# NicoNeureiter/sBayes

Hardware: AMD Instinct MI355X
Metric: log-likelihood evals/sec at 1000 sites x 200 feats x 10 states; 1/2/4/8-GPU chains (higher is better)
Workload: dtype f64; 1 GPU; headline synthetic 1000x200x10, K=5, C=2 (BASELINE.json configs[2]); chains_per_gpu=4096, kernel=packed, log_mode=product, parallelism=1 independent engine(s), one per GPU, no collectives

## Files before the change

sbayes_amd/csrc/sbe_mixture_mfma.hip:

```cpp
#include <algorithm>
#include <cmath>
#include <cstdio>
#include <cstdlib>
#include <type_traits>
#include "sbe_mixture_mfma.hip.h"

#if defined(__HIP_DEVICE_COMPILE__) && !defined(__gfx950__) && !defined(__gfx942__)
#error "sbe_mixture_mfma.hip: the in-kernel final reduction orders relaxed agent-scope atomics by s_waitcnt (gfx942 / gfx950 cache behaviour); not valid for this target"
#endif

namespace sbe {

constexpr int kMfmaRN = kTupleMfmaColsPerPass;

__global__ void k_xt_frags(const uint8_t* __restrict__ state , uint8_t* __restrict__ xt,
                           int N, int F, int S, int Fp, int NT, int KBp) {
    const int64_t u = (int64_t)blockIdx.x * blockDim.x + threadIdx.x;
    if (u >= (int64_t)NT * KBp * 64) return;
    const int l = (int)(u & 63), kb = (int)((u >> 6) % KBp), nt = (int)((u >> 6) / KBp);
    const int col = nt * 32 + (l & 31), f = col / S, s = col - f * S;
    uint32_t w[4] = {0u, 0u, 0u, 0u};
    if (col < F * S) {
        const int n0 = kb * 64 + 32 * (l >> 5);
#pragma unroll
        for (int j = 0; j < 32; ++j) {
            const int n = n0 + 8 * (j >> 3) + (j & 7);
            const int b = j & 3, hi = (j >> 2) & 1;
            if (n < N && state[(int64_t)n * Fp + f] == (uint8_t)s) w[j >> 3] |= 0x2u << (8 * b + 4 * hi);
        }
    }
    reinterpret_cast<uint4*>(xt)[u] = make_uint4(w[0], w[1], w[2], w[3]);
}

__global__ void k_colcount(const uint8_t* __restrict__ state, int32_t* __restrict__ colcount, int32_t* __restrict__ colfeat,
                           int N, int F, int S, int Fp, int NT) {
    const int col = (int)(blockIdx.x * blockDim.x + threadIdx.x);
    if (col >= (NT + 1) * 32) return;
    int c = 0;
    const int f = min(col / S, F - 1);
    if (col < F * S) {
        const int s = col - f * S;
        for (int n = 0; n < N; ++n) c += state[(int64_t)n * Fp + f] == (uint8_t)s;
    }
    colcount[col] = c;
    colfeat[col] = f;
}

__global__ void k_tile_prefix(const int32_t* __restrict__ colcount, int32_t* __restrict__ tile_prefix, int NT) {
    if (threadIdx.x != 0 || blockIdx.x != 0) return;
    int acc = 0;
    for (int t = 0; t <= NT + 1; ++t) {
        tile_prefix[t] = acc;
        if (t <= NT) for (int i = 0; i < 32; ++i) acc += colcount[t * 32 + i];
    }
}

size_t column_tables_bytes(int NT) { return ((size_t)(NT + 1) * 64 + (size_t)NT + 2) * sizeof(int32_t); }
void launch_column_tables(const uint8_t* state, int32_t* out, int N, int F, int S, int Fp, int NT, hipStream_t st) {
    int32_t* colcount = out;
    int32_t* colfeat = out + (size_t)(NT + 1) * 32;
    int32_t* tile_prefix = out + (size_t)(NT + 1) * 64;
    k_colcount<<<(unsigned)(((NT + 1) * 32 + 255) / 256), 256, 0, st>>>(state, colcount, colfeat, N, F, S, Fp, NT);
    k_tile_prefix<<<1, 64, 0, st>>>(colcount, tile_prefix, NT);
}

void launch_xt_frags(const uint8_t* state, uint8_t* xt, int N, int F, int S, int Fp, int NT, int KBp, hipStream_t st) {
    const int64_t units = (int64_t)NT * KBp * 64;
    k_xt_frags<<<(unsigned)((units + 255) / 256), 256, 0, st>>>(state, xt, N, F, S, Fp, NT, KBp);
}

void fine_log_table(double* tab ) {
    for (int i = 0; i < kFineLogEntries; ++i) {
        const long double c = i == 0 ? 1.0L : i == kFineLogEntries - 1 ? 2.0L : 1.0L + (i + 0.5L) / kFineLogEntries;
        const double inv_c = (double)(1.0L / c);
        const long double lc = -logl((long double)inv_c) - (i >= kFineLogSplit ? logl(2.0L) : 0.0L);
        tab[2 * i] = 0.5 * inv_c;
        tab[2 * i + 1] = (i == 0 || i == kFineLogEntries - 1) ? 0.0 : (double)lc;
    }
}

template <int MT, int CT, int GT = 4, int SLB = 4, bool SHARE = false>
__global__ __launch_bounds__(kMfmaThreads, 1) void k_mixture_tuple_mfma(MfmaMixParams p) {
    typedef v16f_t acc_t;
    constexpr int SL = 1 << SLB, TPT = 32 / SL, TPB = MT * TPT;
    constexpr int NK = SL == 16 ? 8 : SL;
    extern __shared__ __align__(16) unsigned char lds_raw[];
    const int lane = threadIdx.x & (kWave - 1);
    const int w = __builtin_amdgcn_readfirstlane((int)(threadIdx.x >> 6));
    const int split = (int)blockIdx.x % p.n_split, sg = (int)blockIdx.x / p.n_split;
    const int KBp = p.KBp;
    constexpr uint32_t tab_off = 0u;
    constexpr uint32_t a_off = kFineLogEntries * 16u;
    const uint32_t a_bytes = (uint32_t)MT * (uint32_t)KBp * 1024u;
    const uint32_t meta_off = a_off + a_bytes;
    const uint32_t red_off = meta_off + (uint32_t)(SL * TPB * sizeof(TupleMeta<CT>));
    const uint32_t lds_base = (uint32_t)(uintptr_t)(__attribute__((address_space(3))) unsigned char*)lds_raw;
    typedef TupleMeta<CT> Meta;
    Meta* meta = reinterpret_cast<Meta*>(lds_raw + meta_off);
    double* red = reinterpret_cast<double*>(lds_raw + red_off);

    auto slot_of = [&](int sl) -> int {
        const int i = sg * SL + sl;
        if (i >= p.n_batch) return -1;
        return p.slot_list ? p.slot_list[i] : p.first_slot + i;
    };

    const int nt_lo = split * p.nt_per_split, nt_hi = min(p.NT, nt_lo + p.nt_per_split);
    constexpr int PF = 4;
    const __amdgpu_buffer_rsrc_t xt_rsrc = __builtin_amdgcn_make_buffer_rsrc(const_cast<uint8_t*>(p.xt), 0, (int)p.xt_bytes, 0x00020000);
    const int lane16 = lane * 16;
    auto tile_off = [&](int nt) -> int { return (nt < nt_hi ? nt : p.NT) * KBp * 1024; };
    auto load_b = [&](int toff, int kb) -> v4i_t {
        const u32x4_t d = __builtin_amdgcn_raw_buffer_load_b128(xt_rsrc, lane16, toff + kb * 1024, 0);
        v4i_t r; r.x = (int)d.x; r.y = (int)d.y; r.z = (int)d.z; r.w = (int)d.w;
        return r;
    };
    v4i_t bq[PF][kMfmaRN];
    {
        const int nt0 = nt_lo + w * kMfmaRN;
#pragma unroll
        for (int i = 0; i < PF; ++i)
#pragma unroll
            for (int r = 0; r < kMfmaRN; ++r) bq[i][r] = load_b(tile_off(nt0 + r), i);
    }

    if (lds_base != 0u) {
        if ((int)threadIdx.x < SL) {
            const int slot = slot_of((int)threadIdx.x);
            if (slot >= 0) {
                p.partials[(int64_t)slot * p.partials_stride + split] = __longlong_as_double(0x7FF8000000000000ll);
                if (p.results) p.results[slot] = __longlong_as_double(0x7FF8000000000000ll);
            }
        }
        return;
    }
    static_assert(!SHARE || (SL == 16 && CT == 2 && MT <= 3), "the shared-operand epilogue: 16 slots, C = 2, <= 6 tuples");
    const uint4* sdesc = reinterpret_cast<const uint4*>(lds_raw + meta_off);
    const uint4* tdesc = reinterpret_cast<const uint4*>(lds_raw + meta_off + SL * 16);
    const int slot_mine = slot_of((int)threadIdx.x & (SL - 1));
    SharedDescIn<SHARE ? TPB : 1> sd_in;
    if constexpr (SHARE) mfma_shared_desc_load<MT, SL>(p, slot_mine, sd_in);
    mfma_phase0<MT, CT, decltype(slot_of), SL, !SHARE>(lds_raw, p, slot_of, tab_off, a_off, meta, KBp, slot_mine);
    if constexpr (SHARE) mfma_shared_desc<MT, SL>(p, sd_in, const_cast<uint4*>(sdesc), const_cast<uint4*>(tdesc));
    __syncthreads();
    bool bad = false;
    if constexpr (SHARE) bad = __builtin_amdgcn_ballot_w64(sdesc[lane & (SL - 1)].w != 0u) != 0ull;

    const int h = lane >> 5, cl = lane & 31;
    double lsum[NK];
    int ksum[NK];
#pragma unroll
    for (int i = 0; i < NK; ++i) { lsum[i] = 0.0; ksum[i] = 0; }
    auto ent_slot = [&](int e) -> int { return ((e & 3) + 8 * (e >> 2) + 4 * h) & (SL - 1); };
    auto ent_tuple = [&](int m, int e) -> int { return m * TPT + (((e & 3) + 8 * (e >> 2) + 4 * h) >> SLB); };
    auto ent_k = [&](int e) -> int { return SL == 16 ? (e & 3) + 4 * ((e >> 2) & 1) : (e & (SL - 1)); };
    int csum = 0;
    uint32_t one_hi = 0x3FF00000u;
    asm volatile("" : "+v"(one_hi));
    const __amdgpu_buffer_rsrc_t pr_rsrc = __builtin_amdgcn_make_buffer_rsrc(const_cast<float*>(p.probs), 0, (int)p.probs_bytes, 0x00020000);
    const __amdgpu_buffer_rsrc_t w_rsrc = __builtin_amdgcn_make_buffer_rsrc(const_cast<float*>(p.wpat), 0, (int)p.wpat_bytes, 0x00020000);
    const uint32_t a_lane = a_off + (uint32_t)lane * 16u;

    auto counts_pass = [&](acc_t (&acc)[MT][kMfmaRN], const int (&toff)[kMfmaRN]) __attribute__((always_inline)) {
        uint32_t a_at[MT];
        v4i_t a_cur[MT];
#pragma unroll
        for (int m = 0; m < MT; ++m) {
            a_at[m] = a_lane + ((uint32_t)m * (uint32_t)KBp) * 1024u;
            asm volatile("" : "+v"(a_at[m]));
            a_cur[m] = *(lds_cv4i_t*)(uintptr_t)a_at[m];
        }
        auto k_group = [&](int kb0, auto first_c) __attribute__((always_inline)) {
            constexpr bool first = decltype(first_c)::value;
#pragma unroll
            for (int i = 0; i < PF; ++i) {
                v4i_t a_nxt[MT];
#pragma unroll
                for (int m = 0; m < MT; ++m) a_nxt[m] = *(lds_cv4i_t*)(uintptr_t)(a_at[m] + (uint32_t)(i + 1) * 1024u);
                const bool refill = !(first && i == 0);
                if (refill) {
#pragma unroll
                    for (int r = 0; r < kMfmaRN; ++r) bq[(i + PF - 1) % PF][r] = load_b(toff[r], kb0 + i + PF - 1);
                }
#pragma unroll
                for (int m = 0; m < MT; ++m)
#pragma unroll
                    for (int r = 0; r < kMfmaRN; ++r) {
                        const v4i_t bx = bq[i][r];
                        const v8i_t a8 = {a_cur[m].x, a_cur[m].y, a_cur[m].z, a_cur[m].w, 0, 0, 0, 0};
                        const v8i_t b8 = {bx.x, bx.y, bx.z, bx.w, 0, 0, 0, 0};
                        const acc_t zero = {0, 0, 0, 0, 0, 0, 0, 0, 0, 0, 0, 0, 0, 0, 0, 0};
                        if (first && i == 0) acc[m][r] = __builtin_amdgcn_mfma_scale_f32_32x32x64_f8f6f4(a8, b8, zero, 4, 4, 0, 0, 0, 0);
                        else acc[m][r] = __builtin_amdgcn_mfma_scale_f32_32x32x64_f8f6f4(a8, b8, acc[m][r], 4, 4, 0, 0, 0, 0);
                    }
#pragma unroll
                for (int m = 0; m < MT; ++m) a_cur[m] = a_nxt[m];
                __builtin_amdgcn_sched_group_barrier(0x100, MT, 0);
                if (refill) __builtin_amdgcn_sched_group_barrier(0x020, kMfmaRN, 0);
                __builtin_amdgcn_sched_group_barrier(0x008, MT * kMfmaRN, 0);
            }
#pragma unroll
            for (int m = 0; m < MT; ++m) a_at[m] += (uint32_t)PF * 1024u;
        };
        k_group(0, std::true_type{});
        for (int kb0 = PF; kb0 < KBp; kb0 += PF) k_group(kb0, std::false_type{});
    };

    constexpr int G = GT;
    constexpr int HQ = 4 / G;
    constexpr int NST = MT * 4 * HQ * kMfmaRN;
    uint32_t col4[kMfmaRN], fw4[kMfmaRN];
    Meta mdq[G];
    float prq[2][G][CT], wrq[2][G][CT];
    auto st_cols = [&](int nt0) {
#pragma unroll
        for (int r = 0; r < kMfmaRN; ++r) {
            const uint32_t colc = (uint32_t)min((nt0 + r) * 32 + cl, p.FS - 1);
            const uint32_t f = colc / (uint32_t)p.S;
            col4[r] = colc * 4u; fw4[r] = f * (uint32_t)(CT * 4);
        }
    };
    auto st_meta = [&](int u) {
        const int mj = u / HQ, half = u % HQ, m = mj >> 2, j = mj & 3;
#pragma unroll
        for (int i = 0; i < G; ++i) {
            const int e = 4 * j + half * G + i;
            mdq[i] = meta[ent_slot(e) * TPB + ent_tuple(m, e)];
        }
    };
    auto st_load = [&](int q) {
        const int r = q % kMfmaRN;
#pragma unroll
        for (int i = 0; i < G; ++i) {
            const uint32_t wo = mdq[i].woff + fw4[r];
            if constexpr (CT == 2) {
                const u32x2_t v2 = __builtin_amdgcn_raw_buffer_load_b64(w_rsrc, (int)wo, 0, 0);
                const uint32_t e0 = v2.x, e1 = v2.y;
                wrq[q & 1][i][0] = __uint_as_float(e0); wrq[q & 1][i][1] = __uint_as_float(e1);
            } else if constexpr (CT == 4) {
                const u32x4_t v4 = __builtin_amdgcn_raw_buffer_load_b128(w_rsrc, (int)wo, 0, 0);
                const uint32_t e0 = v4.x, e1 = v4.y, e2 = v4.z, e3 = v4.w;
                wrq[q & 1][i][0] = __uint_as_float(e0); wrq[q & 1][i][1] = __uint_as_float(e1);
                wrq[q & 1][i][2] = __uint_as_float(e2); wrq[q & 1][i][3] = __uint_as_float(e3);
            } else {
#pragma unroll
                for (int c = 0; c < CT; ++c)
                    wrq[q & 1][i][c] = __builtin_bit_cast(float, __builtin_amdgcn_raw_buffer_load_b32(w_rsrc, (int)(wo + 4u * c), 0, 0));
            }
#pragma unroll
            for (int c = 0; c < CT; ++c)
                prq[q & 1][i][c] = __builtin_bit_cast(float, __builtin_amdgcn_raw_buffer_load_b32(pr_rsrc, (int)(mdq[i].goff[c] + col4[r]), 0, 0));
        }
    };
    auto st_comp = [&](int q, const acc_t (&acc)[MT][kMfmaRN]) __attribute__((always_inline)) {
        const int r = q % kMfmaRN, u = q / kMfmaRN, mj = u / HQ, half = u % HQ, m = mj >> 2, j = mj & 3;
        double vv[G], lg[G], cntd[G];
        int cnt[G];
        bool special = false;
#pragma unroll
        for (int i = 0; i < G; ++i) {
            const float c = acc[m][r][4 * j + half * G + i];
            cnt[i] = (int)c; cntd[i] = (double)c;
            double v = 0.0;
#pragma unroll
            for (int c = 0; c < CT; ++c) {
                const double wc = (double)wrq[q & 1][i][c], pc = (double)prq[q & 1][i][c];
                v = c == 0 ? wc * pc : fma(wc, pc, v);
            }
            vv[i] = v;
            special |= __builtin_amdgcn_class(v, 0x2FF);
        }
        int kx[G];
        tab_log4_n<G>(vv, lg, kx, tab_off, one_hi);
        if (__builtin_expect(__builtin_amdgcn_ballot_w64(special) != 0ull, 0)) {
#pragma unroll
            for (int i = 0; i < G; ++i)
                if (__builtin_amdgcn_class(vv[i], 0x2FF)) { lg[i] = cnt[i] != 0 ? lib_log(vv[i]) : 0.0; kx[i] = kFineLogBias; }
        }
#pragma unroll
        for (int i = 0; i < G; ++i) {
            const int k = ent_k(4 * j + half * G + i);
            lsum[k] = fma(cntd[i], lg[i], lsum[k]);
            ksum[k] = __mul24(cnt[i], kx[i]) + ksum[k];
            asm volatile("" : "+v"(ksum[k]));
            asm volatile("" : "+v"(lsum[k]));
        }
    };

    constexpr int NSS = 8 * MT;
    uint32_t sh_col4[kMfmaRN], sh_fw4[kMfmaRN], col4u = 0;
    uint4 sdq, tdq[2];
    float p0q[2][4], p1r[kMfmaRN];
    uint32_t wr[kMfmaRN][4];
    uint64_t selm[2][2];
    double w0a[kMfmaRN], ua[kMfmaRN], w0b[kMfmaRN], ub[kMfmaRN];
    auto k_slot = [&](int k) -> int { return (k & 3) + 8 * (k >> 2) + 4 * h; };
    auto sh_desc = [&](int k) { sdq = sdesc[k_slot(k)]; };
    auto sh_load = [&]() {
#pragma unroll
        for (int r = 0; r < kMfmaRN; ++r) {
            p1r[r] = __builtin_bit_cast(float, __builtin_amdgcn_raw_buffer_load_b32(pr_rsrc, (int)(sdq.x + sh_col4[r]), 0, 0));
            const u32x2_t va = __builtin_amdgcn_raw_buffer_load_b64(w_rsrc, (int)(sdq.y + sh_fw4[r]), 0, 0);
            const u32x2_t vb = __builtin_amdgcn_raw_buffer_load_b64(w_rsrc, (int)(sdq.z + sh_fw4[r]), 0, 0);
            const uint32_t a0 = va.x, a1 = va.y, b0 = vb.x, b1 = vb.y;
            wr[r][0] = a0; wr[r][1] = a1; wr[r][2] = b0; wr[r][3] = b1;
        }
    };
    auto sh_conv = [&]() {
#pragma unroll
        for (int r = 0; r < kMfmaRN; ++r) {
            const double p1 = (double)p1r[r];
            w0a[r] = (double)__uint_as_float(wr[r][0]); ua[r] = (double)__uint_as_float(wr[r][1]) * p1;
            w0b[r] = (double)__uint_as_float(wr[r][2]); ub[r] = (double)__uint_as_float(wr[r][3]) * p1;
        }
    };
    auto td_read = [&](int q) { tdq[q & 1] = tdesc[k_slot(q / MT) * MT + q % MT]; };
    auto p0_load = [&](int q) {
        const uint4 d = tdq[q & 1];
        const uint32_t o0 = d.x + col4u, o1 = d.y + col4u;
        p0q[q & 1][0] = __builtin_bit_cast(float, __builtin_amdgcn_raw_buffer_load_b32(pr_rsrc, (int)o0, 0, 0));
        p0q[q & 1][1] = __builtin_bit_cast(float, __builtin_amdgcn_raw_buffer_load_b32(pr_rsrc, (int)(o0 + 128u), 0, 0));
        p0q[q & 1][2] = __builtin_bit_cast(float, __builtin_amdgcn_raw_buffer_load_b32(pr_rsrc, (int)o1, 0, 0));
        p0q[q & 1][3] = __builtin_bit_cast(float, __builtin_amdgcn_raw_buffer_load_b32(pr_rsrc, (int)(o1 + 128u), 0, 0));
        selm[q & 1][0] = __builtin_amdgcn_ballot_w64(d.z != 0u);
        selm[q & 1][1] = __builtin_amdgcn_ballot_w64(d.w != 0u);
    };
    auto sh_comp = [&](int q, const acc_t (&acc)[MT][kMfmaRN]) __attribute__((always_inline)) {
        const int k = q / MT, m = q % MT;
        double vv[4], lg[4], cntd[4];
        int cnt[4];
        bool special = false;
#pragma unroll
        for (int i = 0; i < 4; ++i) {
            const int tt = i >> 1, r = i & 1;
            const float c = acc[m][r][4 * ((k >> 2) + 2 * tt) + (k & 3)];
            cnt[i] = (int)c; cntd[i] = (double)c;
            const double p0 = (double)p0q[q & 1][i];
            double v = fma(w0a[r], p0, ua[r]);
            uint64_t keep;
            asm("s_and_saveexec_b64 %1, %2\n\tv_fma_f64 %0, %3, %4, %5\n\ts_mov_b64 exec, %1"
                : "+v"(v), "=&s"(keep) : "s"(selm[q & 1][tt]), "v"(w0b[r]), "v"(p0), "v"(ub[r]) : "scc");
            vv[i] = v;
            special |= __builtin_amdgcn_class(v, 0x2FF);
        }
        int kx[4];
        tab_log4_n<4>(vv, lg, kx, tab_off, one_hi);
        if (__builtin_expect(__builtin_amdgcn_ballot_w64(special) != 0ull, 0)) {
#pragma unroll
            for (int i = 0; i < 4; ++i)
                if (__builtin_amdgcn_class(vv[i], 0x2FF)) { lg[i] = cnt[i] != 0 ? lib_log(vv[i]) : 0.0; kx[i] = kFineLogBias; }
        }
#pragma unroll
        for (int i = 0; i < 4; ++i) {
            lsum[k] = fma(cntd[i], lg[i], lsum[k]);
            ksum[k] = __mul24(cnt[i], kx[i]) + ksum[k];
            asm volatile("" : "+v"(ksum[k]));
            asm volatile("" : "+v"(lsum[k]));
        }
    };

    const __amdgpu_buffer_rsrc_t cc_rsrc = __builtin_amdgcn_make_buffer_rsrc(const_cast<int32_t*>(p.colcount), 0, (p.NT + 1) * 128, 0x00020000);
    auto load_cc = [&](int nt) -> int { return (int)__builtin_amdgcn_raw_buffer_load_b32(cc_rsrc, cl * 4, (nt < nt_hi ? nt : p.NT) * 128, 0); };
    int ccnt[kMfmaRN];
    for (int nt0 = nt_lo + w * kMfmaRN; nt0 < nt_hi; nt0 += kMfmaWaves * kMfmaRN) {
        int toff[kMfmaRN];
#pragma unroll
        for (int r = 0; r < kMfmaRN; ++r) toff[r] = tile_off(nt0 + r);
        const bool first_pass = nt0 == nt_lo + w * kMfmaRN;
        if (!first_pass) {
#pragma unroll
            for (int i = 0; i < PF; ++i)
#pragma unroll
                for (int r = 0; r < kMfmaRN; ++r) bq[i][r] = load_b(toff[r], i);
        }
        if (first_pass) {
#pragma unroll
            for (int r = 0; r < kMfmaRN; ++r) ccnt[r] = load_cc(nt0 + r);
        }
        acc_t acc[MT][kMfmaRN];
        counts_pass(acc, toff);
#pragma unroll
        for (int r = 0; r < kMfmaRN; ++r) {
            csum += ccnt[r];
            ccnt[r] = load_cc(nt0 + kMfmaWaves * kMfmaRN + r);
        }
        if constexpr (SHARE) {
#pragma unroll
            for (int r = 0; r < kMfmaRN; ++r) {
                const uint32_t colc = (uint32_t)min((nt0 + r) * 32 + cl, p.FS - 1);
                sh_col4[r] = colc * 4u; sh_fw4[r] = colc / (uint32_t)p.S * (uint32_t)(CT * 4);
            }
            col4u = (uint32_t)(nt0 * 32 + cl) * 4u;
            sh_desc(0); td_read(0); td_read(1);
            sh_load();
            p0_load(0);
#pragma unroll
            for (int q = 0; q < NSS; ++q) {
                const int k = q / MT, m = q % MT;
                if (m == 0) {
                    sh_conv();
                    if (k + 1 < 8) sh_desc(k + 1);
                }
                if (m == (MT > 1 ? 1 : 0) && k + 1 < 8) sh_load();
                if (q + 1 < NSS) {
                    p0_load(q + 1);
                    if (q + 2 < NSS) td_read(q + 2);
                }
                sh_comp(q, acc);
                __builtin_amdgcn_sched_barrier(0);
            }
        } else {
        st_cols(nt0);
        st_meta(0);
        st_load(0);
#pragma unroll
        for (int q = 0; q < NST; ++q) {
            if (q + 1 < NST) {
                st_load(q + 1);
                if ((q + 2) % kMfmaRN == 0 && q + 2 < NST) st_meta((q + 2) / kMfmaRN);
            }
            st_comp(q, acc);
            __builtin_amdgcn_sched_barrier(0);
        }
        }
    }

#pragma unroll
    for (int i = 0; i < NK; ++i) {
        double v;
        if constexpr (SL == 16) {
            v = fma((double)(ksum[i] - kFineLogBias * csum), 6.93147180559945286227e-01, lsum[i]);
        } else {
            const int ks = ksum[i] + __shfl_xor(ksum[i], 32, 64);
            v = h == 0 ? fma((double)(ks - kFineLogBias * csum), 6.93147180559945286227e-01, lsum[i]) : lsum[i];
        }
#pragma unroll
        for (int off = 16; off >= 1; off >>= 1) v += __shfl_xor(v, off, 64);
        lsum[i] = v;
    }
    if (cl == 0) {
#pragma unroll
        for (int i = 0; i < NK; ++i) {
            if constexpr (SL == 16) {
                const int sl = 8 * (i >> 2) + 4 * h + (i & 3);
                red[(w * 2 + h) * 16 + sl] = lsum[i];
                red[(w * 2 + h) * 16 + (sl ^ 4)] = 0.0;
            } else {
                red[(w * 2 + h) * 16 + i] = lsum[i];
            }
        }
    }
    __syncthreads();
    if (w != 0) return;
    const int my_slot = lane < SL ? slot_of(lane) : -1;
    double total = 0.0;
    if (my_slot >= 0) {
#pragma unroll
        for (int ww = 0; ww < kMfmaWaves; ++ww) { total += red[(ww * 2 + 0) * 16 + lane]; total += red[(ww * 2 + 1) * 16 + lane]; }
    }
    if (bad) total = __longlong_as_double(0x7FF8000000000000ll);
    double* const my_partials = p.partials + (int64_t)max(my_slot, 0) * p.partials_stride;
    if (!p.results) {
        if (my_slot >= 0) my_partials[split] = total;
        return;
    }
    if (p.n_split > 1) {
        if (my_slot >= 0) __hip_atomic_store(my_partials + split, total, __ATOMIC_RELAXED, __HIP_MEMORY_SCOPE_AGENT);
        asm volatile("s_waitcnt vmcnt(0)" ::: "memory");
        unsigned t = 0;
        if (lane == 0) {
            t = __hip_atomic_fetch_add(p.arrive + sg, 1u, __ATOMIC_RELAXED, __HIP_MEMORY_SCOPE_AGENT);
            if (t == (unsigned)p.n_split - 1u) __hip_atomic_store(p.arrive + sg, 0u, __ATOMIC_RELAXED, __HIP_MEMORY_SCOPE_AGENT);
        }
        t = (unsigned)__builtin_amdgcn_readfirstlane((int)t);
        if (t != (unsigned)p.n_split - 1u) return;
        asm volatile("" ::: "memory");
        if (my_slot >= 0) {
            total = 0.0;
            for (int k = 0; k < p.n_split; ++k) total += __hip_atomic_load(my_partials + k, __ATOMIC_RELAXED, __HIP_MEMORY_SCOPE_AGENT);
        }
    }
    if (my_slot >= 0) p.results[my_slot] = total;
    signal_done(p.done);
}

template <int MT, int CT> constexpr int mfma_gt() { return (MT >= 4 || (MT == 3 && CT >= 3)) ? 2 : 4; }

template <int MT, int SLB>
static void launch_mfma_mt(int C, const MfmaMixParams& p, dim3 grid, size_t lds, hipStream_t st) {
    switch (C) {
        case 1: k_mixture_tuple_mfma<MT, 1, mfma_gt<MT, 1>(), SLB><<<grid, kMfmaThreads, lds, st>>>(p); break;
        case 2:
            if constexpr (SLB == 4 && MT <= 3) {
                if (p.shared) { k_mixture_tuple_mfma<MT, 2, mfma_gt<MT, 2>(), SLB, true><<<grid, kMfmaThreads, lds, st>>>(p); break; }
            }
            k_mixture_tuple_mfma<MT, 2, mfma_gt<MT, 2>(), SLB><<<grid, kMfmaThreads, lds, st>>>(p);
            break;
        case 3: k_mixture_tuple_mfma<MT, 3, mfma_gt<MT, 3>(), SLB><<<grid, kMfmaThreads, lds, st>>>(p); break;
        default: k_mixture_tuple_mfma<MT, 4, mfma_gt<MT, 4>(), SLB><<<grid, kMfmaThreads, lds, st>>>(p); break;
    }
}

template <int MT, int CT, int SLB, bool SHARE = false>
static bool allow_lds() {
    const void* fn = reinterpret_cast<const void*>(&k_mixture_tuple_mfma<MT, CT, mfma_gt<MT, CT>(), SLB, SHARE>);
    (void)hipFuncSetAttribute(fn, hipFuncAttributeMaxDynamicSharedMemorySize, (int)kLdsBytes);
    hipFuncAttributes attr{};
    if (hipFuncGetAttributes(&attr, fn) != hipSuccess) { (void)hipGetLastError(); return true; }
    return attr.sharedSizeBytes == 0;
}

template <int SLB>
static bool allow_lds_all() {
    bool ok = true;
    ok &= allow_lds<1, 1, SLB>(); ok &= allow_lds<1, 2, SLB>(); ok &= allow_lds<1, 3, SLB>(); ok &= allow_lds<1, 4, SLB>();
    ok &= allow_lds<2, 1, SLB>(); ok &= allow_lds<2, 2, SLB>(); ok &= allow_lds<2, 3, SLB>(); ok &= allow_lds<2, 4, SLB>();
    ok &= allow_lds<3, 1, SLB>(); ok &= allow_lds<3, 2, SLB>(); ok &= allow_lds<3, 3, SLB>(); ok &= allow_lds<3, 4, SLB>();
    ok &= allow_lds<4, 1, SLB>(); ok &= allow_lds<4, 2, SLB>(); ok &= allow_lds<4, 3, SLB>(); ok &= allow_lds<4, 4, SLB>();
    if constexpr (SLB == 4) {
        ok &= allow_lds<1, 2, SLB, true>(); ok &= allow_lds<2, 2, SLB, true>(); ok &= allow_lds<3, 2, SLB, true>();
    }
    return ok;
}

bool tuple_mfma_shared() {
    static const bool on = [] { const char* v = getenv("SBE_MFMA_SHARED"); return !(v && atoi(v) == 0); }();
    return on;
}

template <int SLB>
static void launch_mfma_slb(int MT, int C, const MfmaMixParams& p, dim3 grid, size_t lds, hipStream_t st) {
    switch (MT) {
        case 1: launch_mfma_mt<1, SLB>(C, p, grid, lds, st); break;
        case 2: launch_mfma_mt<2, SLB>(C, p, grid, lds, st); break;
        case 3: launch_mfma_mt<3, SLB>(C, p, grid, lds, st); break;
        default: launch_mfma_mt<4, SLB>(C, p, grid, lds, st); break;
    }
}

bool launch_tuple_mfma(int C, const MfmaMixParams& p, dim3 grid, size_t lds, hipStream_t st) {
    static const bool no_static_lds = [] { bool ok = allow_lds_all<4>(); ok &= allow_lds_all<2>(); ok &= allow_lds_all<1>(); return ok; }();
    if (!no_static_lds) return false;
    const int SL = p.SL;
    const int MT = (p.KT + 32 / SL - 1) / (32 / SL);
    if (SL == 16) launch_mfma_slb<4>(MT, C, p, grid, lds, st);
    else if (SL == 4) launch_mfma_slb<2>(MT, C, p, grid, lds, st);
    else launch_mfma_slb<1>(MT, C, p, grid, lds, st);
    return true;
}

}
```

sbayes_amd/csrc/sbe_mixture_mfma.hip.h:

```cpp
#pragma once
#include "sbe_mixture.hip.h"

namespace sbe {

typedef int v4i_t __attribute__((ext_vector_type(4)));
typedef int v8i_t __attribute__((ext_vector_type(8)));
typedef float v16f_t __attribute__((ext_vector_type(16)));
typedef __attribute__((address_space(3))) const v4i_t lds_cv4i_t;

constexpr int kMfmaSlots = 16;
constexpr int kMfmaThreads = kMfmaWaves * kWave;

constexpr int kFineLogSplit = 424;
constexpr uint32_t kFineLogCarry = 0x00100000u - ((uint32_t)kFineLogSplit << 10);
constexpr int kFineLogBias = 1023;
template <int G>
__device__ __forceinline__ void tab_log4_n(const double (&v)[G], double (&out)[G], int (&kexp)[G], uint32_t tab, uint32_t one_hi ) {
    f64x2_t e[G];
    double m[G], r[G], q[G];
    uint32_t mant_mask = 0x000FFFFFu;
    asm volatile("" : "+s"(mant_mask));
#pragma unroll
    for (int g = 0; g < G; ++g) {
        const uint32_t hi = (uint32_t)__double2hiint(v[g]);
        e[g] = *(lds_cf64x2_t*)(uintptr_t)(tab + ((hi >> 6) & 0x3FF0u));
        uint32_t mh;
        asm("v_bfi_b32 %0, %1, %2, %3" : "=v"(mh) : "s"(mant_mask), "v"(hi), "v"(one_hi));
        m[g] = __hiloint2double((int)mh, __double2loint(v[g]));
        kexp[g] = (int)((hi + kFineLogCarry) >> 20);
    }
#pragma unroll
    for (int g = 0; g < G; ++g) r[g] = fma(m[g], e[g].x, -0.5);
#pragma unroll
    for (int g = 0; g < G; ++g) q[g] = fma(r[g], -4.0, 8.0 / 3.0);
#pragma unroll
    for (int g = 0; g < G; ++g) q[g] = fma(r[g], q[g], -2.0);
#pragma unroll
    for (int g = 0; g < G; ++g) q[g] = fma(r[g], q[g], 2.0);
#pragma unroll
    for (int g = 0; g < G; ++g) out[g] = fma(r[g], q[g], e[g].y);
}

template <int CT>
struct __attribute__((aligned(CT <= 1 ? 8 : (CT <= 3 ? 16 : 32)))) TupleMeta {
    uint32_t woff;
    uint32_t goff[CT];
};

template <int MT, int CT, typename SlotOf, int SL = kMfmaSlots, bool META = true>
__device__ __forceinline__ void mfma_phase0(unsigned char* lds_raw, const MfmaMixParams& p, const SlotOf& slot_of, uint32_t tab_off,
                                            uint32_t a_off, TupleMeta<CT>* meta, int KBp, int slot_mine) {
    typedef TupleMeta<CT> Meta;
    constexpr int TPT = 32 / SL, TPB = MT * TPT;
    static_assert(SL == 16 || SL == 4 || SL == 2, "slots per block");
    static_assert(kMfmaThreads % SL == 0, "a thread's id units all belong to one slot");
    auto meta_of = [&](int slot, int t, uint32_t pat, const uint32_t (&g)[CT]) -> Meta {
        Meta md;
        md.woff = p.wpat_ones_off;
#pragma unroll
        for (int c = 0; c < CT; ++c) md.goff[c] = p.probs_ones_off;
        if (slot >= 0 && t < p.KT && pat != 0xFFu) {
            md.woff = (uint32_t)(((int64_t)slot * p.wpat_stride + (int64_t)pat * p.F * CT) * 4);
#pragma unroll
            for (int c = 0; c < CT; ++c)
                if ((int)g[c] < p.Gtot) md.goff[c] = (uint32_t)(((int64_t)slot * p.probs_stride + (int64_t)g[c] * p.FS) * 4);
        }
        return md;
    };
    constexpr bool PERM = TPB <= 8;
    constexpr uint32_t kNoTuple = PERM ? 0x0C0C0C0Cu : 0xFFFFFFFFu;
    const int n_units = SL * KBp * 2;
    constexpr int UB = 2;
    uint32_t d[UB][8];
    auto load_ids = [&](int u0) {
#pragma unroll
        for (int k = 0; k < UB; ++k) {
            const int u = u0 + k * kMfmaThreads;
            const int n0 = (u / SL) * 32;
            const int slot = u < n_units ? slot_mine : -1;
#pragma unroll
            for (int i = 0; i < 8; ++i) {
                d[k][i] = kNoTuple;
                if (slot >= 0 && n0 + 4 * i + 4 <= p.Np)
                    d[k][i] = *reinterpret_cast<const uint32_t*>(p.tid + (int64_t)slot * p.tid_stride + n0 + 4 * i);
            }
        }
    };
    auto emit = [&](int u0) {
#pragma unroll
        for (int k = 0; k < UB; ++k) {
            const int u = u0 + k * kMfmaThreads;
            if (u >= n_units) break;
            const int sl = u % SL, hk = u / SL;
            const int kb = hk >> 1, h = hk & 1;
#pragma unroll 8
            for (int t = 0; t < TPB; ++t) {
                uint4 o;
                uint32_t* ov = reinterpret_cast<uint32_t*>(&o);
#pragma unroll
                for (int wv = 0; wv < 4; ++wv) {
                    if constexpr (PERM) {
                        const uint64_t lut = 0x02ull << (8 * (t & 7));
                        const uint32_t lo = __builtin_amdgcn_perm((uint32_t)(lut >> 32), (uint32_t)lut, d[k][2 * wv]);
                        const uint32_t hi = __builtin_amdgcn_perm((uint32_t)(lut >> 32), (uint32_t)lut, d[k][2 * wv + 1]);
                        ov[wv] = lo | (hi << 4);
                        continue;
                    }
                    uint32_t eq[2];
#pragma unroll
                    for (int q = 0; q < 2; ++q) {
                        const uint32_t x = d[k][2 * wv + q] ^ ((uint32_t)t * 0x01010101u);
                        const uint32_t nz = ((x & 0x7F7F7F7Fu) + 0x7F7F7F7Fu) | x;
                        eq[q] = (~nz >> 7) & 0x01010101u;
                    }
                    ov[wv] = (eq[0] << 1) | (eq[1] << 5);
                }
                const uint32_t fl = (uint32_t)(h * 32 + (t % TPT) * SL + sl);
                *reinterpret_cast<uint4*>(lds_raw + a_off + (((uint32_t)(t / TPT) * (uint32_t)KBp + (uint32_t)kb) * 64u + fl) * 16u) = o;
            }
        }
    };
    const int u_first = (int)threadIdx.x;
    load_ids(u_first);
    constexpr int LT = (2 * kFineLogEntries + kMfmaThreads - 1) / kMfmaThreads;
    double lt[LT];
#pragma unroll
    for (int k = 0; k < LT; ++k) {
        const int i = (int)threadIdx.x + k * kMfmaThreads;
        lt[k] = i < 2 * kFineLogEntries ? reinterpret_cast<const double*>(p.logtab)[i] : 0.0;
    }
    const bool has_meta = META && (int)threadIdx.x < SL * TPB;
    const int m_sl = (int)threadIdx.x / TPB, m_t = (int)threadIdx.x % TPB;
    const int m_slot = has_meta ? slot_of(m_sl) : -1;
    uint32_t m_pat = 0xFFu, m_g[CT];
#pragma unroll
    for (int c = 0; c < CT; ++c) m_g[c] = 0xFFFFFFFFu;
    if (m_slot >= 0) {
        m_pat = p.tuple_p[(int64_t)m_slot * p.tuple_p_stride + m_t];
#pragma unroll
        for (int c = 0; c < CT; ++c) m_g[c] = p.tuple_g[(int64_t)m_slot * p.tuple_g_stride + m_t * kMaxComponents + c];
    }
    if (has_meta) meta[m_sl * TPB + m_t] = meta_of(m_slot, m_t, m_pat, m_g);
    (void)meta;
#pragma unroll
    for (int k = 0; k < LT; ++k) {
        const int i = (int)threadIdx.x + k * kMfmaThreads;
        if (i < 2 * kFineLogEntries) reinterpret_cast<double*>(lds_raw + tab_off)[i] = lt[k];
    }
    for (int u0 = u_first; u0 < n_units; u0 += UB * kMfmaThreads) {
        if (u0 != u_first) load_ids(u0);
        emit(u0);
    }
}

template <int TPB>
struct SharedDescIn {
    int slot;
    uint32_t pat[TPB], g0[TPB], g1[TPB];
};

template <int MT, int SL>
__device__ __forceinline__ void mfma_shared_desc_load(const MfmaMixParams& p, int slot, SharedDescIn<MT * 32 / SL>& in) {
    constexpr int TPB = MT * 32 / SL;
    static_assert(SL == 16 && TPB <= kMaxTuples, "the shared-operand form has 16 slots of <= 8 tuples");
    if ((int)threadIdx.x >= SL) return;
    in.slot = slot;
    const uint8_t* const tp = p.tuple_p + (int64_t)max(slot, 0) * p.tuple_p_stride;
    const uint16_t* const tg = p.tuple_g + (int64_t)max(slot, 0) * p.tuple_g_stride;
#pragma unroll
    for (int t = 0; t < TPB; ++t) {
        in.pat[t] = tp[t];
        in.g0[t] = tg[t * kMaxComponents + 0];
        in.g1[t] = tg[t * kMaxComponents + 1];
    }
}

template <int MT, int SL>
__device__ __forceinline__ void mfma_shared_desc(const MfmaMixParams& p, const SharedDescIn<MT * 32 / SL>& in, uint4* sdesc, uint4* tdesc) {
    constexpr int TPB = MT * 32 / SL;
    if ((int)threadIdx.x >= SL) return;
    const int sl = (int)threadIdx.x, slot = in.slot;
    const uint32_t (&g0)[TPB] = in.g0, (&g1)[TPB] = in.g1;
    uint32_t pat[TPB];
#pragma unroll
    for (int t = 0; t < TPB; ++t) pat[t] = (slot >= 0 && t < p.KT) ? in.pat[t] : 0xFFu;
    auto goff = [&](uint32_t g) -> uint32_t {
        return (int)g < p.Gtot ? (uint32_t)(((int64_t)slot * p.probs_stride + (int64_t)g * p.FS) * 4) : p.probs_ones_off;
    };
    uint32_t goff1 = p.probs_ones_off, wa = p.wpat_ones_off, wb = p.wpat_ones_off, bad = 0u;
    uint32_t go0[TPB], sel[TPB];
    bool any = false;
#pragma unroll
    for (int t = 0; t < TPB; ++t) {
        go0[t] = p.probs_ones_off; sel[t] = 0u;
        if (pat[t] == 0xFFu) continue;
        go0[t] = goff(g0[t]);
        const uint32_t wo = (uint32_t)(((int64_t)slot * p.wpat_stride + (int64_t)pat[t] * p.F * 2) * 4), g1o = goff(g1[t]);
        if (!any) { any = true; goff1 = g1o; wa = wb = wo; }
        if (g1o != goff1) bad = 1u;
        if (wo != wa) {
            if (wb == wa) wb = wo;
            else if (wo != wb) bad = 1u;
            sel[t] = 1u;
        }
    }
    sdesc[sl] = make_uint4(goff1, wa, wb, bad);
#pragma unroll
    for (int m = 0; m < MT; ++m) tdesc[sl * MT + m] = make_uint4(go0[2 * m], go0[2 * m + 1], sel[2 * m], sel[2 * m + 1]);
}

}
```

Measured before the change: 76.79 million evals/s.

## Split epilogue log into LDS lookup and series stages, software-pipelined across half-groups

Splits the table-log computation into a separate LDS lookup stage and a polynomial series stage. Work now moves in half-groups, so the lookup for the next group is issued before the series of the current one, with global loads prefetched further ahead. Partial sched barriers replace full ones. The aim is to hide LDS and global load latency in the epilogue, at the cost of more live registers and more complex scheduling.

```diff
diff --git a/sbayes_amd/csrc/sbe_mixture_mfma.hip b/sbayes_amd/csrc/sbe_mixture_mfma.hip
--- a/sbayes_amd/csrc/sbe_mixture_mfma.hip
+++ b/sbayes_amd/csrc/sbe_mixture_mfma.hip
@@ -209,9 +209,10 @@
     constexpr int G = GT;
     constexpr int HQ = 4 / G;
     constexpr int NST = MT * 4 * HQ * kMfmaRN;
+    constexpr int GS = G / 2, NG = 2 * NST;
     uint32_t col4[kMfmaRN], fw4[kMfmaRN];
     Meta mdq[G];
-    float prq[2][G][CT], wrq[2][G][CT];
+    float prq[2][GS][CT], wrq[2][GS][CT];
     auto st_cols = [&](int nt0) {
 #pragma unroll
         for (int r = 0; r < kMfmaRN; ++r) {
@@ -228,68 +229,89 @@
             mdq[i] = meta[ent_slot(e) * TPB + ent_tuple(m, e)];
         }
     };
-    auto st_load = [&](int q) {
-        const int r = q % kMfmaRN;
-#pragma unroll
-        for (int i = 0; i < G; ++i) {
-            const uint32_t wo = mdq[i].woff + fw4[r];
+    auto st_load = [&](int g) {
+        const int r = (g >> 1) % kMfmaRN, gi = g & 1;
+#pragma unroll
+        for (int i = 0; i < GS; ++i) {
+            const Meta& md = mdq[gi * GS + i];
+            const uint32_t wo = md.woff + fw4[r];
             if constexpr (CT == 2) {
                 const u32x2_t v2 = __builtin_amdgcn_raw_buffer_load_b64(w_rsrc, (int)wo, 0, 0);
                 const uint32_t e0 = v2.x, e1 = v2.y;
-                wrq[q & 1][i][0] = __uint_as_float(e0); wrq[q & 1][i][1] = __uint_as_float(e1);
+                wrq[g & 1][i][0] = __uint_as_float(e0); wrq[g & 1][i][1] = __uint_as_float(e1);
             } else if constexpr (CT == 4) {
                 const u32x4_t v4 = __builtin_amdgcn_raw_buffer_load_b128(w_rsrc, (int)wo, 0, 0);
                 const uint32_t e0 = v4.x, e1 = v4.y, e2 = v4.z, e3 = v4.w;
-                wrq[q & 1][i][0] = __uint_as_float(e0); wrq[q & 1][i][1] = __uint_as_float(e1);
-                wrq[q & 1][i][2] = __uint_as_float(e2); wrq[q & 1][i][3] = __uint_as_float(e3);
+                wrq[g & 1][i][0] = __uint_as_float(e0); wrq[g & 1][i][1] = __uint_as_float(e1);
+                wrq[g & 1][i][2] = __uint_as_float(e2); wrq[g & 1][i][3] = __uint_as_float(e3);
             } else {
 #pragma unroll
                 for (int c = 0; c < CT; ++c)
-                    wrq[q & 1][i][c] = __builtin_bit_cast(float, __builtin_amdgcn_raw_buffer_load_b32(w_rsrc, (int)(wo + 4u * c), 0, 0));
+                    wrq[g & 1][i][c] = __builtin_bit_cast(float, __builtin_amdgcn_raw_buffer_load_b32(w_rsrc, (int)(wo + 4u * c), 0, 0));
             }
 #pragma unroll
             for (int c = 0; c < CT; ++c)
-                prq[q & 1][i][c] = __builtin_bit_cast(float, __builtin_amdgcn_raw_buffer_load_b32(pr_rsrc, (int)(mdq[i].goff[c] + col4[r]), 0, 0));
-        }
-    };
-    auto st_comp = [&](int q, const acc_t (&acc)[MT][kMfmaRN]) __attribute__((always_inline)) {
+                prq[g & 1][i][c] = __builtin_bit_cast(float, __builtin_amdgcn_raw_buffer_load_b32(pr_rsrc, (int)(md.goff[c] + col4[r]), 0, 0));
+        }
+    };
+#define SBE_EPI_FENCE() __builtin_amdgcn_sched_barrier(0x0074)
+    double pv[2][2];
+    f64x2_t pe[2][2];
+    auto grp_series = [&](int g, auto ne, const float* c, const int* k) __attribute__((always_inline)) {
+        constexpr int NE = decltype(ne)::value;
+        double vv[NE], lg[NE], cntd[NE];
+        f64x2_t ee[NE];
+        int cnt[NE], kx[NE];
+        bool special = false;
+#pragma unroll
+        for (int i = 0; i < NE; ++i) {
+            vv[i] = pv[g & 1][i]; ee[i] = pe[g & 1][i];
+            cnt[i] = (int)c[i]; cntd[i] = (double)c[i];
+            special |= __builtin_amdgcn_class(vv[i], 0x2FF);
+        }
+        tab_log_series<NE>(vv, ee, lg, kx, one_hi);
+        if (__builtin_expect(__builtin_amdgcn_ballot_w64(special) != 0ull, 0)) {
+            int bias = kFineLogBias;
+            asm volatile("" : "+v"(bias));
+#pragma unroll
+            for (int i = 0; i < NE; ++i)
+                if (__builtin_amdgcn_class(vv[i], 0x2FF)) { lg[i] = cnt[i] != 0 ? lib_log(vv[i]) : 0.0; kx[i] = bias; }
+        }
+#pragma unroll
+        for (int i = 0; i < NE; ++i) {
+            lsum[k[i]] = fma(cntd[i], lg[i], lsum[k[i]]);
+            ksum[k[i]] = __mul24(cnt[i], kx[i]) + ksum[k[i]];
+            asm volatile("" : "+v"(ksum[k[i]]));
+            asm volatile("" : "+v"(lsum[k[i]]));
+        }
+    };
+    auto st_look = [&](int g) __attribute__((always_inline)) {
+#pragma unroll
+        for (int i = 0; i < GS; ++i) {
+            double v = 0.0;
+#pragma unroll
+            for (int c = 0; c < CT; ++c) {
+                const double wc = (double)wrq[g & 1][i][c], pc = (double)prq[g & 1][i][c];
+                v = c == 0 ? wc * pc : fma(wc, pc, v);
+            }
+            pv[g & 1][i] = v;
+            pe[g & 1][i] = tab_log_lookup(v, tab_off);
+        }
+    };
+    auto st_series = [&](int g, const acc_t (&acc)[MT][kMfmaRN]) __attribute__((always_inline)) {
+        const int q = g >> 1, gi = g & 1;
         const int r = q % kMfmaRN, u = q / kMfmaRN, mj = u / HQ, half = u % HQ, m = mj >> 2, j = mj & 3;
-        double vv[G], lg[G], cntd[G];
-        int cnt[G];
-        bool special = false;
-#pragma unroll
-        for (int i = 0; i < G; ++i) {
-            const float c = acc[m][r][4 * j + half * G + i];
-            cnt[i] = (int)c; cntd[i] = (double)c;
-            double v = 0.0;
-#pragma unroll
-            for (int c = 0; c < CT; ++c) {
-                const double wc = (double)wrq[q & 1][i][c], pc = (double)prq[q & 1][i][c];
-                v = c == 0 ? wc * pc : fma(wc, pc, v);
-            }
-            vv[i] = v;
-            special |= __builtin_amdgcn_class(v, 0x2FF);
-        }
-        int kx[G];
-        tab_log4_n<G>(vv, lg, kx, tab_off, one_hi);
-        if (__builtin_expect(__builtin_amdgcn_ballot_w64(special) != 0ull, 0)) {
-#pragma unroll
-            for (int i = 0; i < G; ++i)
-                if (__builtin_amdgcn_class(vv[i], 0x2FF)) { lg[i] = cnt[i] != 0 ? lib_log(vv[i]) : 0.0; kx[i] = kFineLogBias; }
-        }
-#pragma unroll
-        for (int i = 0; i < G; ++i) {
-            const int k = ent_k(4 * j + half * G + i);
-            lsum[k] = fma(cntd[i], lg[i], lsum[k]);
-            ksum[k] = __mul24(cnt[i], kx[i]) + ksum[k];
-            asm volatile("" : "+v"(ksum[k]));
-            asm volatile("" : "+v"(lsum[k]));
-        }
+        const int e0 = 4 * j + half * G + GS * gi;
+        float c[GS];
+        int k[GS];
+#pragma unroll
+        for (int i = 0; i < GS; ++i) { c[i] = acc[m][r][e0 + i]; k[i] = ent_k(e0 + i); }
+        grp_series(g, std::integral_constant<int, GS>{}, c, k);
     };
 
     constexpr int NSS = 8 * MT;
     uint32_t sh_col4[kMfmaRN], sh_fw4[kMfmaRN], col4u = 0;
-    uint4 sdq, tdq[2];
+    uint4 sdq, tdq;
     float p0q[2][4], p1r[kMfmaRN];
     uint32_t wr[kMfmaRN][4];
     uint64_t selm[2][2];
@@ -306,6 +328,12 @@
             wr[r][0] = a0; wr[r][1] = a1; wr[r][2] = b0; wr[r][3] = b1;
         }
     };
+    auto sh_next = [&](int k1) {
+        if (k1 < 8) {
+            sh_load();
+            if (k1 + 1 < 8) sh_desc(k1 + 1);
+        }
+    };
     auto sh_conv = [&]() {
 #pragma unroll
         for (int r = 0; r < kMfmaRN; ++r) {
@@ -314,9 +342,9 @@
             w0b[r] = (double)__uint_as_float(wr[r][2]); ub[r] = (double)__uint_as_float(wr[r][3]) * p1;
         }
     };
-    auto td_read = [&](int q) { tdq[q & 1] = tdesc[k_slot(q / MT) * MT + q % MT]; };
+    auto td_read = [&](int q) { tdq = tdesc[k_slot(q / MT) * MT + q % MT]; };
     auto p0_load = [&](int q) {
-        const uint4 d = tdq[q & 1];
+        const uint4 d = tdq;
         const uint32_t o0 = d.x + col4u, o1 = d.y + col4u;
         p0q[q & 1][0] = __builtin_bit_cast(float, __builtin_amdgcn_raw_buffer_load_b32(pr_rsrc, (int)o0, 0, 0));
         p0q[q & 1][1] = __builtin_bit_cast(float, __builtin_amdgcn_raw_buffer_load_b32(pr_rsrc, (int)(o0 + 128u), 0, 0));
@@ -325,38 +353,25 @@
         selm[q & 1][0] = __builtin_amdgcn_ballot_w64(d.z != 0u);
         selm[q & 1][1] = __builtin_amdgcn_ballot_w64(d.w != 0u);
     };
-    auto sh_comp = [&](int q, const acc_t (&acc)[MT][kMfmaRN]) __attribute__((always_inline)) {
-        const int k = q / MT, m = q % MT;
-        double vv[4], lg[4], cntd[4];
-        int cnt[4];
-        bool special = false;
-#pragma unroll
-        for (int i = 0; i < 4; ++i) {
-            const int tt = i >> 1, r = i & 1;
-            const float c = acc[m][r][4 * ((k >> 2) + 2 * tt) + (k & 3)];
-            cnt[i] = (int)c; cntd[i] = (double)c;
-            const double p0 = (double)p0q[q & 1][i];
+    auto sh_look = [&](int g) __attribute__((always_inline)) {
+        const int q = g >> 1, tt = g & 1;
+#pragma unroll
+        for (int r = 0; r < 2; ++r) {
+            const double p0 = (double)p0q[q & 1][2 * tt + r];
             double v = fma(w0a[r], p0, ua[r]);
             uint64_t keep;
             asm("s_and_saveexec_b64 %1, %2\n\tv_fma_f64 %0, %3, %4, %5\n\ts_mov_b64 exec, %1"
                 : "+v"(v), "=&s"(keep) : "s"(selm[q & 1][tt]), "v"(w0b[r]), "v"(p0), "v"(ub[r]) : "scc");
-            vv[i] = v;
-            special |= __builtin_amdgcn_class(v, 0x2FF);
-        }
-        int kx[4];
-        tab_log4_n<4>(vv, lg, kx, tab_off, one_hi);
-        if (__builtin_expect(__builtin_amdgcn_ballot_w64(special) != 0ull, 0)) {
-#pragma unroll
-            for (int i = 0; i < 4; ++i)
-                if (__builtin_amdgcn_class(vv[i], 0x2FF)) { lg[i] = cnt[i] != 0 ? lib_log(vv[i]) : 0.0; kx[i] = kFineLogBias; }
-        }
-#pragma unroll
-        for (int i = 0; i < 4; ++i) {
-            lsum[k] = fma(cntd[i], lg[i], lsum[k]);
-            ksum[k] = __mul24(cnt[i], kx[i]) + ksum[k];
-            asm volatile("" : "+v"(ksum[k]));
-            asm volatile("" : "+v"(lsum[k]));
-        }
+            pv[g & 1][r] = v;
+            pe[g & 1][r] = tab_log_lookup(v, tab_off);
+        }
+    };
+    auto sh_series = [&](int g, const acc_t (&acc)[MT][kMfmaRN]) __attribute__((always_inline)) {
+        const int q = g >> 1, tt = g & 1, k = q / MT, m = q % MT;
+        const int e = 4 * ((k >> 2) + 2 * tt) + (k & 3);
+        const float c[2] = {acc[m][0][e], acc[m][1][e]};
+        const int kk[2] = {k, k};
+        grp_series(g, std::integral_constant<int, 2>{}, c, kk);
     };
 
     const __amdgpu_buffer_rsrc_t cc_rsrc = __builtin_amdgcn_make_buffer_rsrc(const_cast<int32_t*>(p.colcount), 0, (p.NT + 1) * 128, 0x00020000);
@@ -391,36 +406,56 @@
                 sh_col4[r] = colc * 4u; sh_fw4[r] = colc / (uint32_t)p.S * (uint32_t)(CT * 4);
             }
             col4u = (uint32_t)(nt0 * 32 + cl) * 4u;
-            sh_desc(0); td_read(0); td_read(1);
+            sh_desc(0); td_read(0);
             sh_load();
+            if (MT == 1) sh_desc(1);
             p0_load(0);
+            td_read(1);
+            p0_load(1);
+            td_read(2);
+            sh_conv();
+            if (MT == 1) sh_next(1);
+            sh_look(0);
 #pragma unroll
             for (int q = 0; q < NSS; ++q) {
                 const int k = q / MT, m = q % MT;
-                if (m == 0) {
-                    sh_conv();
-                    if (k + 1 < 8) sh_desc(k + 1);
+                if (MT > 1 && k + 1 < 8) {
+                    if (m == 0) sh_desc(k + 1);
+                    if (m == 1) sh_load();
                 }
-                if (m == (MT > 1 ? 1 : 0) && k + 1 < 8) sh_load();
+                sh_look(2 * q + 1);
+                if (q + 2 < NSS) {
+                    p0_load(q + 2);
+                    if (q + 3 < NSS) td_read(q + 3);
+                }
+                SBE_EPI_FENCE();
+                sh_series(2 * q, acc);
                 if (q + 1 < NSS) {
-                    p0_load(q + 1);
-                    if (q + 2 < NSS) td_read(q + 2);
+                    if ((q + 1) % MT == 0) {
+                        sh_conv();
+                        if (MT == 1) sh_next(k + 2);
+                    }
+                    sh_look(2 * q + 2);
                 }
-                sh_comp(q, acc);
-                __builtin_amdgcn_sched_barrier(0);
+                SBE_EPI_FENCE();
+                sh_series(2 * q + 1, acc);
             }
         } else {
         st_cols(nt0);
         st_meta(0);
         st_load(0);
-#pragma unroll
-        for (int q = 0; q < NST; ++q) {
-            if (q + 1 < NST) {
-                st_load(q + 1);
-                if ((q + 2) % kMfmaRN == 0 && q + 2 < NST) st_meta((q + 2) / kMfmaRN);
-            }
-            st_comp(q, acc);
-            __builtin_amdgcn_sched_barrier(0);
+        st_load(1);
+        st_look(0);
+        st_load(2);
+#pragma unroll
+        for (int g = 0; g < NG; ++g) {
+            if (g + 1 < NG) st_look(g + 1);
+            if (g + 3 < NG) {
+                st_load(g + 3);
+                if ((g + 4) % (2 * kMfmaRN) == 0 && g + 4 < NG) st_meta((g + 4) / (2 * kMfmaRN));
+            }
+            SBE_EPI_FENCE();
+            st_series(g, acc);
         }
         }
     }
diff --git a/sbayes_amd/csrc/sbe_mixture_mfma.hip.h b/sbayes_amd/csrc/sbe_mixture_mfma.hip.h
--- a/sbayes_amd/csrc/sbe_mixture_mfma.hip.h
+++ b/sbayes_amd/csrc/sbe_mixture_mfma.hip.h
@@ -14,16 +14,19 @@
 constexpr int kFineLogSplit = 424;
 constexpr uint32_t kFineLogCarry = 0x00100000u - ((uint32_t)kFineLogSplit << 10);
 constexpr int kFineLogBias = 1023;
+__device__ __forceinline__ f64x2_t tab_log_lookup(double v, uint32_t tab) {
+    const uint32_t hi = (uint32_t)__double2hiint(v);
+    return *(lds_cf64x2_t*)(uintptr_t)(tab + ((hi >> 6) & 0x3FF0u));
+}
 template <int G>
-__device__ __forceinline__ void tab_log4_n(const double (&v)[G], double (&out)[G], int (&kexp)[G], uint32_t tab, uint32_t one_hi ) {
-    f64x2_t e[G];
+__device__ __forceinline__ void tab_log_series(const double (&v)[G], const f64x2_t (&e)[G], double (&out)[G], int (&kexp)[G],
+                                               uint32_t one_hi ) {
     double m[G], r[G], q[G];
     uint32_t mant_mask = 0x000FFFFFu;
     asm volatile("" : "+s"(mant_mask));
 #pragma unroll
     for (int g = 0; g < G; ++g) {
         const uint32_t hi = (uint32_t)__double2hiint(v[g]);
-        e[g] = *(lds_cf64x2_t*)(uintptr_t)(tab + ((hi >> 6) & 0x3FF0u));
         uint32_t mh;
         asm("v_bfi_b32 %0, %1, %2, %3" : "=v"(mh) : "s"(mant_mask), "v"(hi), "v"(one_hi));
         m[g] = __hiloint2double((int)mh, __double2loint(v[g]));
```

Result: no change. 77.16 million evals/s (median of 6 runs) (+0.5%).
